# amazon-science/instruct-video-to-video

Hardware: AMD Instinct MI355X
Metric: denoised video-frames/sec (16f@256x384, 50 DDIM steps) (higher is better)
Workload: dtype fp16; 1 GPU; C2: 1 clip/step = VAE-encode + 50 DDIM steps (3-way CFG, text 7.5 / video 1.5) + VAE-decode, 16 frames @ 256x384, random-init full-width UNet+VAE; 5 independent clips in flight per GPU (stacked into every UNet launch, B = 3 x clips); frames=16, height=256, width=384, ddim_steps=50, clips_per_gpu=5, parallelism=clip-parallel x1, one all_gather, hip_graph=True, cfg_branch_streams=False, concurrent_clips=5, clip_mode=stacked, driver_mode=False, full=False

## Files before the change

### include/insv2v_hip.h

```cpp
#ifndef INSV2V_HIP_H
#define INSV2V_HIP_H

#include <stdint.h>

#ifdef __cplusplus
extern "C" {
#endif

typedef void* insv2v_stream_t;

#define INSV2V_OK 0
#define INSV2V_EINVAL (-1)
#define INSV2V_EUNSUPPORTED (-2)

#define INSV2V_ACT_NONE 0
#define INSV2V_ACT_SILU 1
#define INSV2V_ACT_GEGLU 2
#define INSV2V_ACT_QUICK_GELU 3

#define INSV2V_ACT_RELU 4
#define INSV2V_ACT_SIGMOID 5
#define INSV2V_ACT_TANH 6

#define INSV2V_MODE_LINEAR 0
// ... 26 lines not shown
    int32_t NB, IH, IW, OH, OW, Cin;
    int32_t stride, pad_t, pad_l, upsample;
    int32_t batch;
    int32_t tile;
    int32_t split_k;
    float alpha;
    const float* gn_ab;
    int32_t gn_images_per_sample;
    int32_t gn_silu;
    float* stats_out;
    float* stats_scratch;
    int32_t stats_parts;
    float ln_eps;
    int64_t w_group_stride;
    int32_t w_group_rows;
    int32_t reserved0;
} insv2v_gemm_desc;
int insv2v_gemm(const insv2v_gemm_desc* d, insv2v_stream_t stream);
int64_t insv2v_set_operand_window(int64_t bytes);
int insv2v_gemm_stats_parts(const insv2v_gemm_desc* d);
int insv2v_conv3x3_fuses_groupnorm(const insv2v_gemm_desc* d);
#define INSV2V_PLAN_NONE 0
#define INSV2V_PLAN_TILE 1
#define INSV2V_PLAN_HALO 2
#define INSV2V_PLAN_Q8 3
#define INSV2V_PLAN_R8 4
#define INSV2V_PLAN_W4 5
typedef struct insv2v_gemm_plan_t {
    int32_t rc;
    int32_t family;
    int32_t variant;
// ... 186 lines not shown
    int32_t grid;
    int32_t lds_bytes;
    int32_t rows_per_wg;
    int32_t ntiles;
    int32_t ragged;
} insv2v_attention_plan_t;
int insv2v_attention_plan(const insv2v_attention_desc* d, int32_t cus, insv2v_attention_plan_t* out);

int insv2v_embed_tokens(const int64_t* ids, const void* tok, const void* pos, void* out, int32_t rows, int32_t L,
                        int32_t C, int32_t vocab, insv2v_stream_t stream);

int insv2v_softmax_rows(const void* x, void* y, int64_t ldx, int64_t ldy, int32_t rows, int32_t cols,
                        float scale, insv2v_stream_t stream);
int insv2v_softmax_rows_padded(const void* x, void* y, int64_t ldx, int64_t ldy, int32_t rows, int32_t cols, int32_t valid,
                               float scale, insv2v_stream_t stream);

int insv2v_timestep_embedding(const float* t, void* out, int32_t batch, int32_t dim, float shift,
                              insv2v_stream_t stream);

int insv2v_tap_gather(const float* y9, int64_t ld9, const float* bias, float* out, int64_t ldo, int32_t NB, int32_t H, int32_t W,
                      int32_t cout, insv2v_stream_t stream);

int insv2v_build_unet_input(const float* latent, const float* img_cond, void* out, float* t_out,
                            float timestep, int32_t nbranch, int32_t F, int32_t h, int32_t w, int32_t ldo,
                            int64_t branch_rows, int32_t t_stride, insv2v_stream_t stream);

typedef struct insv2v_step_desc {
    const float* eps_in;
    const float* latent;
    const float* latent_ref;
// ... 251 lines not shown
```

### instruct-video-to-video_amd/csrc/gemm_plan.h

```cpp
#pragma once
#include <stdint.h>
#include <algorithm>
#include "../../include/insv2v_hip.h"

constexpr int GEMM_BK = 64;
constexpr int W4_BK = 32;

struct gemm_switches {
    int r8 = 1;
    int r8_stats = 1;
    int q8_min_n = 256;
    int persistent = 1;
    int r8_geglu = 1;
    int r8_cim = 1;
    int halo_legacy_map = 0;
    int r8_dephase = 0;
    int w4_wgs = 2, w4_delay = -1;
};
const gemm_switches& insv2v_gemm_switches();

static inline void gemm_defaults(insv2v_gemm_desc& d) { if (d.batch <= 0) d.batch = 1; if (d.alpha == 0.f) d.alpha = 1.f; }
static inline bool misaligned16(const void* p) { return ((uintptr_t)p & 15) != 0; }
static inline bool beyond_2g(int64_t bytes) { return bytes >= ((int64_t)1 << 31); }

// ... 146 lines not shown
    const int64_t nparts = (total + per - 1) / per;
    return ((total + nparts - 1) / nparts + unit - 1) / unit * unit;
}

static inline insv2v_gemm_desc window_part(const insv2v_gemm_desc& f, int64_t u0, int64_t nu) {
    const bool conv = f.mode == INSV2V_MODE_CONV3X3;
    const int64_t opix = conv ? (int64_t)f.OH * f.OW : 1, ipix = conv ? (int64_t)f.IH * f.IW : 1, esz = f.c_fp32 ? 4 : 2;
    const int64_t r_in = u0 * ipix, r_out = u0 * opix;
    insv2v_gemm_desc d = f;
    d.a = (const char*)f.a + r_in * f.lda * 2;
    if (f.k_split) d.a2 = (const char*)f.a2 + r_in * f.lda2 * 2;
    d.c = (char*)f.c + r_out * f.ldc * esz;
    if (f.residual) d.residual = (const char*)f.residual + r_out * f.ldr * 2;
    if (f.row_stats) d.row_stats = f.row_stats + r_out * 2;
    if (f.w_group_rows > 0) d.w = (const char*)f.w + (r_out / f.w_group_rows) * f.w_group_stride * 2;
    if (f.row_bias && f.rb_mod <= 0) d.row_bias = f.row_bias + (r_out / f.rows_per_group) * f.ld_rb;
    if (conv && f.gn_ab) d.gn_ab = f.gn_ab + (u0 / f.gn_images_per_sample) * (int64_t)f.Cin * 2;
    d.M = (int32_t)(nu * opix); if (conv) d.NB = (int32_t)nu;
    return d;
}
static inline void stats_finished(insv2v_gemm_desc& d) { d.row_stats = d.stats_scratch; d.stats_parts = 0; }

static inline int validate_gemm(const insv2v_gemm_desc& d, int stats_width) {
    if (!d.a || !d.w || !d.c || d.M <= 0 || d.N <= 0 || d.K <= 0) return INSV2V_EINVAL;
    if ((d.K & 7) || (d.lda & 7) || (d.ldw & 7)) return INSV2V_EINVAL;
    if (misaligned16(d.a) || misaligned16(d.w)) return INSV2V_EINVAL;
    if (d.k_split && (!d.a2 || (d.k_split % GEMM_BK) || (d.lda2 & 7) || misaligned16(d.a2))) return INSV2V_EINVAL;
    if (d.row_bias && d.rows_per_group <= 0) return INSV2V_EINVAL;
    if (d.row_stats && (!d.col_sum || d.batch > 1)) return INSV2V_EINVAL;
    if (d.stats_parts < 0 || (d.stats_parts > 0 && (!d.row_stats || !d.stats_scratch))) return INSV2V_EINVAL;
    if (d.stats_out && stats_width == 0) return INSV2V_EUNSUPPORTED;
    if (d.act == INSV2V_ACT_GEGLU && (d.N % 64)) return INSV2V_EINVAL;
    if (d.act < 0 || d.act > INSV2V_ACT_TANH) return INSV2V_EINVAL;
    if (d.w_group_rows < 0 || (d.w_group_rows > 0 && (d.w_group_rows % 256 || d.w_group_stride <= 0))) return INSV2V_EINVAL;
    if (d.w_group_rows > 0 && (d.mode != INSV2V_MODE_LINEAR || d.batch > 1 || d.c_fp32 || d.act != INSV2V_ACT_NONE || d.residual || d.row_bias || d.row_stats ||
                               d.stats_out || d.k_split || d.split_k > 1 || d.K < 256 || (d.N % 256 && d.N % 320)))
        return INSV2V_EUNSUPPORTED;
    if (d.gn_ab && (d.mode != INSV2V_MODE_CONV3X3 || d.gn_images_per_sample <= 0 || d.upsample)) return INSV2V_EINVAL;
    if (d.mode == INSV2V_MODE_CONV3X3) {
        if (d.Cin <= 0 || (d.Cin % GEMM_BK) || d.K != 9 * d.Cin) return INSV2V_EINVAL;
        if ((long)d.NB * d.OH * d.OW != d.M || d.stride < 1) return INSV2V_EINVAL;
        if (d.upsample && (d.stride != 1 || d.pad_t != 1 || d.pad_l != 1 || (d.OH != 2 * d.IH && d.OH != 2 * d.IH - 1) || (d.OW != 2 * d.IW && d.OW != 2 * d.IW - 1)))
            return INSV2V_EINVAL;
    } else if (d.mode != INSV2V_MODE_LINEAR) {
        return INSV2V_EUNSUPPORTED;
    }
    return beyond_2g((int64_t)d.N * d.ldw * 2) ? INSV2V_EUNSUPPORTED : 0;
}

static inline int engine_tile_code(int family) { return family == INSV2V_PLAN_R8 ? 240 : family == INSV2V_PLAN_Q8 ? 230 : 210; }
// ... 25 lines not shown
        const int64_t per = units_per_part(d, window), total = conv ? d.NB : d.M;
        if (per <= 0) return refuse(INSV2V_EUNSUPPORTED);
        const bool finalize = d.stats_parts > 0;
        if (finalize) stats_finished(d);
        const insv2v_gemm_plan_t first = plan_gemm(window_part(d, 0, per), cus, window, sw);
        if (first.rc) return refuse(first.rc);
        const int32_t stats_w_ = p.stats_width, fuse = p.gn_fuse;
        p = first;
        p.stats_width = stats_w_; p.gn_fuse = fuse; p.ln_finalize = finalize;
        p.parts = (int32_t)((total + per - 1) / per);
        p.units_per_part = (int32_t)per;
        return p;
    }
    if (d.w_group_rows > 0) {
        const int64_t groups = ((int64_t)d.M + d.w_group_rows - 1) / d.w_group_rows;
        if (beyond_2g(groups * d.w_group_stride * 2)) return refuse(INSV2V_EUNSUPPORTED);
        if (cus <= 0) return refuse(INSV2V_EINVAL);
        const bool r_ok = d.N % 320 == 0, q_ok = d.N % 256 == 0;
        const pingpong_cost c = pingpong_costs(d, cus);
        const bool use_r = d.tile / 10 == 24 ? true : d.tile / 10 == 23 ? false : (r_ok && (!q_ok || c.r8 <= c.q8));
        if (use_r ? !r_ok : !q_ok) return refuse(INSV2V_EUNSUPPORTED);
        if (const int rc = engine(use_r ? R8 : Q8)) return refuse(rc);
        return p;
    }
    if (d.tile >= 200 && d.tile <= 206) return refuse(INSV2V_EUNSUPPORTED);
    if ((d.tile >= 230 && d.tile <= 249) || (d.tile >= 210 && d.tile <= 221)) {
        const int family = d.tile >= 240 ? R8 : d.tile >= 230 ? Q8 : W4;
        if (d.split_k > 1 || (d.stats_out && family != R8)) return refuse(INSV2V_EUNSUPPORTED);
        d.split_k = 1;
        if (const int rc = engine(family, d.tile - engine_tile_code(family))) return refuse(rc);
        return p;
// ... 44 lines not shown
```

### instruct-video-to-video_amd/csrc/gemm_q8.hip

```cpp
#include "common.h"
#include "gemm_dma.h"
#include "gemm_plan.h"
#include <type_traits>

namespace {

constexpr int HALF_B = 128 * 128;
constexpr int RING_B = 8 * HALF_B;
constexpr int PARK_B = 5 * 1024;
constexpr int LDS_B = RING_B + 2 * PARK_B;
constexpr int STAMP_B = 8 * 512;

#ifndef Q8_MID_SPREAD
#define Q8_MID_SPREAD 1
#endif
#define SB() __builtin_amdgcn_sched_barrier(0)
#define BARRIER() do { SB(); __builtin_amdgcn_s_barrier(); SB(); } while (0)

typedef unsigned uint4v __attribute__((ext_vector_type(4)));
__device__ __forceinline__ unsigned pack_h2(float x, float y) {
    typedef float f2_t __attribute__((ext_vector_type(2)));
    const f2_t v = {x, y};
    return __builtin_bit_cast(unsigned, __builtin_convertvector(v, half2v));
}
// ... 102 lines not shown
    auto stage_piece = [&](auto part_c, auto buf_c, int i) {
        constexpr int PART = decltype(part_c)::value, BUF = decltype(buf_c)::value;
        char* dst = smem + (PART * 2 + BUF) * HALF_B + wid * 1024 + i * 8192;
        if (PART >= 2) dma16(rW, woff[(PART - 2) * 2 + i], cur.k0 * 2 + (int)cur.wbase, dst);
        else dma16(cur.second ? rA2 : rA, aoff[PART * 2 + i], cur.soffA, dst);
    };
    auto stage = [&](auto part_c, auto buf_c) { stage_piece(part_c, buf_c, 0); stage_piece(part_c, buf_c, 1); };
    auto row_group = [&](int m) { int g = m / p.rows_per_group; if (p.rb_mod > 0) g %= p.rb_mod; return g; };
    auto stage_park = [&](int pb, int bm0, int bn0) {
        char* dst = smem + RING_B + pb * PARK_B + wid * 1024;
        if (wid == 0) {
            const int n = bn0 + lane * 4;
            dma16(rBias, (p.bias && n < p.N) ? (unsigned)(n * 4) : OOB_OFFSET, 0, dst);
        } else if (wid == 1) {
            const int n = bn0 + lane * 4;
            dma16(rCs, (ln && n < p.N) ? (unsigned)(n * 4) : OOB_OFFSET, 0, dst);
        } else if (wid == 2 || wid == 3) {
            const int m = bm0 + (wid - 2) * 128 + lane * 2;
            dma16(rSt, (ln && m < p.M) ? (unsigned)(m * 8) : OOB_OFFSET, 0, dst);
        } else if (wid == 4) {
            const int n = bn0 + lane * 4;
            const int g = p.row_bias ? row_group(bm0) : 0;
            dma16(rRb, (p.row_bias && n < p.N) ? (unsigned)((g * (int)p.ld_rb + n) * 4) : OOB_OFFSET, 0, dst);
        }
    };

    const int l15 = lane & 15, lq = lane >> 4, fsw = l15 >> 1;
    const char* aRd[2];
    const char* wRd[2];
#pragma unroll
    for (int kb = 0; kb < 2; ++kb) {
// ... 292 lines not shown
```

### instruct-video-to-video_amd/csrc/gemm_r8.hip

```cpp
#include "common.h"
#include "gemm_dma.h"
#include "gemm_plan.h"
#include <type_traits>

namespace {

constexpr int BM = 256, BN = 320;
constexpr int AH_B = 128 * 128;
constexpr int WB_B = 64 * 128;
constexpr int W_BASE = 4 * AH_B;
constexpr int RING_B = 4 * AH_B + 10 * WB_B;
constexpr int PK_BIAS = 0, PK_CS = 2048, PK_ST = 4096, PK_RB = 6144, PARK_B = 8192;
constexpr int LDS_B = RING_B + 2 * PARK_B;

#ifndef R8_MID_SPREAD
#define R8_MID_SPREAD 1
#endif
#define SB() __builtin_amdgcn_sched_barrier(0)
#define BARRIER() do { SB(); __builtin_amdgcn_s_barrier(); SB(); } while (0)

typedef unsigned uint4v __attribute__((ext_vector_type(4)));
typedef unsigned uint2v __attribute__((ext_vector_type(2)));
__device__ __forceinline__ unsigned pack_h2(float x, float y) {
    typedef float f2_t __attribute__((ext_vector_type(2)));
// ... 155 lines not shown
        } else {
            dma16(rW, min(woff + (unsigned)(PB * 32 * (int)p.ldw * 2), wmax), cur.k0 * 2 + (int)cur.wbase, dst);
        }
    };
    auto row_group = [&](int m) { int g = m / p.rows_per_group; if (p.rb_mod > 0) g %= p.rb_mod; return g; };
    auto stage_park = [&](int pb, int bm0, int bn0) {
        char* park = smem + RING_B + pb * PARK_B;
        const srd_t rBias = make_srd(p.bias ? (const void*)p.bias : p.w), rCs = make_srd(ln ? (const void*)p.col_sum : p.w),
                    rSt = make_srd(ln ? (const void*)p.row_stats : p.w), rRb = make_srd(p.row_bias ? (const void*)p.row_bias : p.w);
        const int hi = wid & 1;
        const int n = bn0 + hi * 256 + lane * 4;
        const bool okn = n < p.N && (hi == 0 || lane < 16);
        if (wid < 2) {
            dma16(rBias, (p.bias && okn) ? (unsigned)(n * 4) : OOB_OFFSET, 0, park + PK_BIAS + hi * 1024);
        } else if (wid < 4) {
            dma16(rCs, (ln && okn) ? (unsigned)(n * 4) : OOB_OFFSET, 0, park + PK_CS + hi * 1024);
        } else if (wid < 6) {
            const int m = bm0 + hi * 128 + lane * 2;
            dma16(rSt, (ln && m < p.M) ? (unsigned)(m * 8) : OOB_OFFSET, 0, park + PK_ST + hi * 1024);
        } else {
            const int g = p.row_bias ? row_group(bm0) : 0;
            dma16(rRb, (p.row_bias && okn) ? (unsigned)((g * (int)p.ld_rb + n) * 4) : OOB_OFFSET, 0, park + PK_RB + hi * 1024);
        }
    };

    const int l15 = lane & 15, lq = lane >> 4, fsw = l15 >> 1;
    const char* aRd[2];
    const char* wRd[2];
#pragma unroll
    for (int kb = 0; kb < 2; ++kb) {
        const int co = ((kb * 4 + lq) ^ fsw) * 16;
// ... 356 lines not shown
```

### instruct-video-to-video_amd/csrc/norm.hip

```cpp
#include "common.h"
#include "norm_plan.h"
#include <cstdlib>

struct Moments {
    float n, mean, m2;
};
static_assert(sizeof(Moments) == GN_MOMENTS_BYTES, "norm_plan.h restates the size");
__device__ __forceinline__ Moments merge(Moments a, Moments b) {
    if (b.n == 0.f) return a;
    if (a.n == 0.f) return b;
    Moments r;
    r.n = a.n + b.n;
    float d = b.mean - a.mean;
    r.mean = a.mean + d * (b.n / r.n);
    r.m2 = a.m2 + b.m2 + d * d * (a.n * b.n / r.n);
    return r;
}

__device__ __forceinline__ half8 load8(const half_t* x, const half_t* x2, int64_t ldx, int64_t ldx2, int C1,
                                       int64_t row, int c0) {
    const half_t* p = (c0 < C1) ? x + row * ldx + c0 : x2 + row * ldx2 + (c0 - C1);
    return *(const half8*)p;
}

// ... 597 lines not shown
    if (!x || !y || rows <= 0 || cols <= 0 || (cols & 7) || (ldx & 7) || (ldy & 7)) return INSV2V_EINVAL;
    if (scale < 0.f) return INSV2V_EINVAL;
    hipLaunchKernelGGL(softmax_rows_kernel<false>, dim3(rows), dim3(256), 0, as_stream(stream), (const half_t*)x,
                       (half_t*)y, ldx, ldy, cols, cols, scale);
    return launch_status();
}

extern "C" int insv2v_softmax_rows_padded(const void* x, void* y, int64_t ldx, int64_t ldy, int32_t rows, int32_t cols, int32_t valid,
                                          float scale, insv2v_stream_t stream) {
    if (!x || !y || rows <= 0 || cols <= 0 || (cols & 7) || (ldx & 7) || (ldy & 7) || ldx < cols || ldy < cols) return INSV2V_EINVAL;
    if (valid <= 0 || valid > cols || scale < 0.f) return INSV2V_EINVAL;
    hipLaunchKernelGGL(softmax_rows_kernel<true>, dim3(rows), dim3(256), 0, as_stream(stream), (const half_t*)x,
                       (half_t*)y, ldx, ldy, cols, valid, scale);
    return launch_status();
}
```

### instruct-video-to-video_amd/insv2v/_lib.py

```python
import ctypes as C
import os

import torch

ABI_VERSION = 15
_HERE = os.path.dirname(os.path.abspath(__file__))
LIB_PATH = os.environ.get("INSV2V_LIB", os.path.join(_HERE, "libinsv2v_hip.so"))

c_i32, c_i64, c_f32, c_p = C.c_int32, C.c_int64, C.c_float, C.c_void_p


class GemmDesc(C.Structure):
    _fields_ = [("a", c_p), ("a2", c_p), ("w", c_p), ("c", c_p), ("bias", c_p), ("row_bias", c_p), ("residual", c_p),
                ("row_stats", c_p), ("col_sum", c_p),
                ("lda", c_i64), ("lda2", c_i64), ("ldw", c_i64), ("ldc", c_i64), ("ldr", c_i64), ("ld_rb", c_i64),
                ("a_bs", c_i64), ("w_bs", c_i64), ("c_bs", c_i64), ("r_bs", c_i64),
                ("workspace", c_p), ("workspace_bytes", c_i64),
                ("M", c_i32), ("N", c_i32), ("K", c_i32), ("k_split", c_i32), ("rows_per_group", c_i32),
                ("rb_mod", c_i32), ("act", c_i32), ("c_fp32", c_i32), ("mode", c_i32),
                ("NB", c_i32), ("IH", c_i32), ("IW", c_i32), ("OH", c_i32), ("OW", c_i32), ("Cin", c_i32),
                ("stride", c_i32), ("pad_t", c_i32), ("pad_l", c_i32), ("upsample", c_i32),
                ("batch", c_i32), ("tile", c_i32), ("split_k", c_i32), ("alpha", c_f32),
                ("gn_ab", c_p), ("gn_images_per_sample", c_i32), ("gn_silu", c_i32),
                ("stats_out", c_p), ("stats_scratch", c_p), ("stats_parts", c_i32), ("ln_eps", c_f32),
                ("w_group_stride", c_i64), ("w_group_rows", c_i32), ("reserved0", c_i32)]


class GemmPlan(C.Structure):
    _fields_ = [(n, c_i32) for n in ("rc", "family", "variant", "ring", "tw_shift", "cim", "split_k", "ln_finalize", "splitk_reduce", "stats_width",
                                     "gn_fuse", "parts", "units_per_part", "forced_tile")]


class WinogradInDesc(C.Structure):
    _fields_ = [("x", c_p), ("x2", c_p), ("gn_ab", c_p), ("v", c_p), ("ldx", c_i64), ("ldx2", c_i64), ("v_group_rows", c_i64),
                ("NB", c_i32), ("H", c_i32), ("W", c_i32), ("C", c_i32), ("C1", c_i32), ("gn_images_per_sample", c_i32), ("gn_silu", c_i32), ("upsample", c_i32)]


class WinogradOutDesc(C.Structure):
    _fields_ = [("m", c_p), ("bias", c_p), ("row_bias", c_p), ("residual", c_p), ("y", c_p), ("m_group_rows", c_i64),
                ("ldr", c_i64), ("ldy", c_i64), ("ld_rb", c_i64), ("NB", c_i32), ("H", c_i32), ("W", c_i32), ("Cout", c_i32), ("rows_per_group", c_i32), ("upsample", c_i32)]
# ... 151 lines not shown
    "insv2v_tattn_attn": (c_i32, [C.POINTER(TattnDesc), c_p]),
    "insv2v_tattn_attn_stream_elems": (c_i64, [c_i32, c_i32, c_i32]),
    "insv2v_xattn_fused": (c_i32, [C.POINTER(XattnDesc), c_p]),
    "insv2v_xattn_stream_elems": (c_i64, [c_i32, c_i32, c_i32]),
    "insv2v_xattn_attn": (c_i32, [C.POINTER(XattnDesc), c_p]),
    "insv2v_xattn_attn_stream_elems": (c_i64, [c_i32, c_i32, c_i32]),
    "insv2v_groupnorm": (c_i32, [C.POINTER(GroupNormDesc), c_p]),
    "insv2v_groupnorm_plan": (c_i32, [C.POINTER(GroupNormDesc), C.POINTER(GroupNormPlan)]),
    "insv2v_layernorm": (c_i32, [C.POINTER(LayerNormDesc), c_p]),
    "insv2v_layernorm_stats": (c_i32, [c_p, c_p, c_i64, c_i32, c_i32, c_f32, c_p]),
    "insv2v_attention": (c_i32, [C.POINTER(AttentionDesc), c_p]),
    "insv2v_attention_plan": (c_i32, [C.POINTER(AttentionDesc), c_i32, C.POINTER(AttentionPlan)]),
    "insv2v_embed_tokens": (c_i32, [c_p, c_p, c_p, c_p, c_i32, c_i32, c_i32, c_i32, c_p]),
    "insv2v_softmax_rows": (c_i32, [c_p, c_p, c_i64, c_i64, c_i32, c_i32, c_f32, c_p]),
    "insv2v_softmax_rows_padded": (c_i32, [c_p, c_p, c_i64, c_i64, c_i32, c_i32, c_i32, c_f32, c_p]),
    "insv2v_timestep_embedding": (c_i32, [c_p, c_p, c_i32, c_i32, c_f32, c_p]),
    "insv2v_build_unet_input": (c_i32, [c_p, c_p, c_p, c_p, c_f32, c_i32, c_i32, c_i32, c_i32, c_i32, c_i64, c_i32, c_p]),
    "insv2v_cfg_step": (c_i32, [C.POINTER(StepDesc), c_p]),
    "insv2v_cfg_step_ms": (c_i32, [C.POINTER(MStepDesc), c_p]),
    "insv2v_cfg_step_mask": (c_i32, [C.POINTER(MaskStepDesc), c_p]),
    "insv2v_mask_to_latent": (c_i32, [c_p, c_p, c_i32, c_i32, c_i32, c_i32, c_p]),
    "insv2v_composite": (c_i32, [c_p, c_p, c_p, c_p, c_i32, c_i32, c_i32, c_p]),
    "insv2v_add_noise": (c_i32, [c_p, c_p, c_p, c_i64, c_f32, c_f32, c_p]),
    "insv2v_cfg_stats": (c_i32, [c_p, c_p, c_i32, c_i32, c_i32, c_f32, c_f32, c_i64, c_p]),
    "insv2v_warp_image": (c_i32, [c_p, c_p, c_p, c_i32, c_i32, c_i32, c_i32, c_p]),
    "insv2v_tap_gather": (c_i32, [c_p, c_i64, c_p, c_p, c_i64, c_i32, c_i32, c_i32, c_i32, c_p]),
    "insv2v_resize_flow": (c_i32, [c_p, c_p, c_i32, c_i32, c_i32, c_i32, c_i32, c_p]),
    "insv2v_flow_correction": (c_i32, [c_p, c_p, c_p, c_p, c_p, c_i32, c_i32, c_i32, c_i32, c_f32, c_f32, c_p]),
    "insv2v_nchw_to_nhwc_f16": (c_i32, [c_p, c_p, c_i32, c_i32, c_i32, c_i32, c_i32, c_f32, c_p]),
    "insv2v_nhwc_to_nchw_f32": (c_i32, [c_p, c_i32, c_p, c_i32, c_i32, c_i32, c_i32, c_i32, c_f32, c_p]),
# ... 60 lines not shown
```

### instruct-video-to-video_amd/insv2v/inference.py

```python
import os
import weakref

import torch

from . import ops
from .fused import check_operand_windows
from .rng import stream_id, STEP, MASK, WINDOW_BITS, STEP_BITS
from .schedulers import DDIMScheduler, DDPMScheduler, DPMSolverMultistepScheduler, strength_to_start
from .flow_utils import resize_flow


class GraphedUNet:

    def __init__(self, unet, B, F, H, W, ctx_len, use_graph=True, branch_streams=False, cfg_clips=0):
        dev = unet.device
        self.branch_streams = branch_streams and B > 1
        self.cfg_clips = cfg_clips if (cfg_clips > 0 and B == 3 * cfg_clips and not self.branch_streams) else 0
        self._streams = None
        try:
            self._unet = weakref.ref(unet)
        except TypeError:
            self._unet = lambda u=unet: u
        self.key = (B, F, H, W, ctx_len)
        self.x_in = torch.zeros((B * F * H * W, unet.in_pad), device=dev, dtype=torch.float16)
# ... 4 lines not shown
        self.eps = None
        self.start = 0
        self._ws = [ops.new_workspace(dev) for _ in range(B if self.branch_streams else 1)]

    @property
    def unet(self):
        u = self._unet()
        if u is None:
            raise RuntimeError("GraphedUNet: its UNet has been garbage collected")
        return u

    def set_context(self, ctx):
        kvs, L = self.unet.project_context(ctx)
        assert L == self.key[4] and ctx.shape[0] == self.key[0]
        if self.kvs is None:
            self.kvs = [tuple(torch.zeros_like(t) for t in kv) if isinstance(kv, tuple) else torch.zeros_like(kv) for kv in kvs]
        for dst, src in zip(self.kvs, kvs):
            for d, s_ in zip(dst, src) if isinstance(dst, tuple) else ((dst, src),):
                d.copy_(s_)

    def _forward(self):
        B, F, H, W, L = self.key
        if not self.branch_streams:
            with ops.workspace(self._ws[0]):
                return self.unet.forward_cl(self.x_in, self.t, self.kvs, L, B, F, H, W, start=self.start, cfg_clips=self.cfg_clips)
        if self._streams is None:
            self._streams = [torch.cuda.Stream() for _ in range(B)]
        main = torch.cuda.current_stream()
        rows = F * H * W
        outs = [None] * B
        for b, st in enumerate(self._streams):
            st.wait_stream(main)
            with torch.cuda.stream(st), ops.workspace(self._ws[b]):
                kvs = [(kv[0][b * L:(b + 1) * L], kv[1][b:b + 1]) if isinstance(kv, tuple) else kv[b * L:(b + 1) * L] for kv in self.kvs]
                outs[b] = self.unet.forward_cl(self.x_in[b * rows:(b + 1) * rows], self.t[b:b + 1], kvs, L, 1, F, H, W,
                                               start=self.start)
        for st in self._streams:
            main.wait_stream(st)
        return torch.cat(outs, 0)

    def run(self):
        if not self.use_graph:
            return self._forward()
        if self.graph is None:
            s = torch.cuda.Stream()
            s.wait_stream(torch.cuda.current_stream())
            with torch.cuda.stream(s):
                self._forward()
            torch.cuda.current_stream().wait_stream(s)
# ... 567 lines not shown
```

### instruct-video-to-video_amd/insv2v/ops.py

```python
import ctypes as C

import math
import os
import torch

from . import _lib
from .rng import as_int64
from ._lib import GemmDesc, GroupNormDesc, LayerNormDesc, AttentionDesc, StepDesc, MStepDesc, MaskStepDesc, MaskTrackDesc, FfnDesc, RowLinDesc, TattnDesc, XattnDesc, WinogradInDesc, WinogradOutDesc, check

ACT_NONE, ACT_SILU, ACT_GEGLU, ACT_QUICK_GELU = 0, 1, 2, 3
ACT_RELU, ACT_SIGMOID, ACT_TANH = 4, 5, 6
EW_RELU, EW_ADD_RELU, EW_TANH, EW_GRU_RH, EW_GRU_OUT = 1, 2, 3, 4, 5
_byref = C.byref


def _stream():
    return torch.cuda.current_stream().cuda_stream


_REC = None


def set_launch_recorder(rec):
    global _REC
# ... 66 lines not shown


class RowStats:
    __slots__ = ("parts", "nparts", "eps")

    def __init__(self, parts, nparts, eps):
        self.parts, self.nparts, self.eps = parts, nparts, eps


_STATS_PARTS_CACHE = {}


def gemm(a, w, bias=None, *, a2=None, act=ACT_NONE, residual=None, row_bias=None, rows_per_group=0, rb_mod=0,
         row_stats=None, col_sum=None, emit_stats=False, ln_eps=1e-5,
         out=None, out_fp32=False, alpha=1.0, tile=0, split_k=0, batch=1, a_bs=0, w_bs=0, c_bs=0, r_bs=0,
         M=None, N=None, K=None, lda=None, ldw=None, ldc=None):
    lib = _lib.load()
    _req(a, torch.float16, "gemm.a"), _req(w, torch.float16, "gemm.w")
    M = a.shape[0] if M is None else M
    N = w.shape[0] if N is None else N
    k1 = a.shape[1]
    K = (k1 + (a2.shape[1] if a2 is not None else 0)) if K is None else K
    n_out = N // 2 if act == ACT_GEGLU else N
    if out is None:
        shape = (M, n_out) if batch == 1 else (batch, M, n_out)
        out = torch.empty(shape, device=a.device, dtype=torch.float32 if out_fp32 else torch.float16)
    d = GemmDesc()
    d.a, d.w, d.c = a.data_ptr(), w.data_ptr(), out.data_ptr()
    d.lda = a.stride(0) if lda is None else lda
    d.ldw = w.stride(0) if ldw is None else ldw
    d.ldc = (out.stride(-2) if ldc is None else ldc)
# ... 7 lines not shown
    if residual is not None:
        d.residual, d.ldr = _req(residual, torch.float16, "gemm.residual").data_ptr(), residual.stride(-2)
    scratch = None
    if isinstance(row_stats, RowStats):
        d.row_stats = row_stats.parts.data_ptr()
        d.stats_parts, d.ln_eps = row_stats.nparts, row_stats.eps
        scratch = torch.empty((M, 2), device=a.device, dtype=torch.float32)
        d.stats_scratch = scratch.data_ptr()
        d.col_sum = _req(col_sum, torch.float32, "gemm.col_sum").data_ptr()
    elif row_stats is not None:
        d.row_stats = _req(row_stats, torch.float32, "gemm.row_stats").data_ptr()
        d.col_sum = _req(col_sum, torch.float32, "gemm.col_sum").data_ptr()
    d.rb_mod = rb_mod
    d.M, d.N, d.K, d.act, d.c_fp32, d.alpha, d.tile = M, N, K, act, int(out.dtype == torch.float32), alpha, tile
    d.batch, d.a_bs, d.w_bs, d.c_bs, d.r_bs = batch, a_bs, w_bs, c_bs, r_bs
    if batch == 1:
        ws = _workspace(a.device)
        d.workspace, d.workspace_bytes, d.split_k = ws.data_ptr(), ws.numel() * 4, split_k
    stats = None
    if emit_stats:
        key = (M, N, K, d.lda, d.ldc, d.ldr, residual is not None, act, tile, out.dtype, a.data_ptr() % 16, out.data_ptr() % 16, batch, split_k,
               residual.data_ptr() % 16 if residual is not None else 0,
               row_bias is not None, rows_per_group, d.ld_rb, rb_mod, a2 is not None, row_stats is not None)
        nparts = _STATS_PARTS_CACHE.get(key)
        if nparts is None:
            nparts = _STATS_PARTS_CACHE[key] = int(lib.insv2v_gemm_stats_parts(_byref(d)))
        if nparts > 0:
            stats = RowStats(torch.empty((nparts, M, 2), device=a.device, dtype=torch.float32), nparts, ln_eps)
            d.stats_out = stats.parts.data_ptr()
    with _timed("gemm_kernel", 2.0 * M * N * K * batch, ("lin", M, N, K, batch, act, residual is not None)):
        rc = lib.insv2v_gemm(_byref(d), _stream())
        if rc == -2 and stats is not None:
            stats, d.stats_out = None, None
            rc = lib.insv2v_gemm(_byref(d), _stream())
        check(rc, "insv2v_gemm")
    del scratch
    if emit_stats:
        return out, (stats if stats is not None else layernorm_stats(out, ln_eps))
# ... 436 lines not shown


def softmax_rows(x, scale=1.0, valid=None):
    lib = _lib.load()
    _req(x, torch.float16, "softmax.x")
    x2 = x.reshape(-1, x.shape[-1])
    if valid is not None and valid != x2.shape[1]:
        check(lib.insv2v_softmax_rows_padded(x2.data_ptr(), x2.data_ptr(), x2.stride(0), x2.stride(0), x2.shape[0], x2.shape[1], valid,
                                             scale, _stream()), "insv2v_softmax_rows_padded")
        return x
    check(lib.insv2v_softmax_rows(x2.data_ptr(), x2.data_ptr(), x2.stride(0), x2.stride(0), x2.shape[0], x2.shape[1],
                                  scale, _stream()), "insv2v_softmax_rows")
    return x


def timestep_embedding(t_dev, dim, shift=0.0):
    lib = _lib.load()
    _req(t_dev, torch.float32, "timestep")
    out = torch.empty((t_dev.shape[0], dim), device=t_dev.device, dtype=torch.float16)
    check(lib.insv2v_timestep_embedding(t_dev.data_ptr(), out.data_ptr(), t_dev.shape[0], dim, shift, _stream()),
          "insv2v_timestep_embedding")
    return out


def build_unet_input(latent, img_cond, out, t_out, timestep, nbranch, branch_rows=0, t_stride=0):
    lib = _lib.load()
    F, _, h, w = latent.shape[-4:]
    check(lib.insv2v_build_unet_input(_req(latent, torch.float32, "latent").data_ptr(),
                                      _req(img_cond, torch.float32, "img_cond").data_ptr(), out.data_ptr(),
                                      _ptr(t_out), float(timestep), nbranch, F, h, w, out.shape[-1], branch_rows, t_stride, _stream()),
# ... 587 lines not shown
```

### instruct-video-to-video_amd/insv2v/unet.py

```python
import math
import os

import torch

from . import ops
from . import fused
from .fused import check_operand_windows, pack_ffn_stream, pack_linear_stream, pack_tattn_stream, pack_tattn_qkv_stream

CPAD = 64
FUSE_GN = os.environ.get("INSV2V_FUSE_GN", "0") != "0"
FUSE_FFN = os.environ.get("INSV2V_FUSE_FFN", "1") != "0"
FUSE_FFN_POST = os.environ.get("INSV2V_FUSE_FFN_POST", "1") != "0"
DEDUP_CFG = os.environ.get("INSV2V_DEDUP_CFG", "1") != "0"
WINOGRAD = os.environ.get("INSV2V_WINOGRAD", "1") != "0"
WINOGRAD_MIN_CIN = int(os.environ.get("INSV2V_WINOGRAD_MIN_CIN", "1280"))
WINOGRAD_MIN_ROWS = int(os.environ.get("INSV2V_WINOGRAD_MIN_ROWS", "4608"))
WINOGRAD_UP_MIN_CIN = int(os.environ.get("INSV2V_WINOGRAD_UP_MIN_CIN", "640"))
MERGE_FF2_POST = os.environ.get("INSV2V_MERGE_FF2_POST", "1") != "0"
NARROW_CONV_OUT = os.environ.get("INSV2V_NARROW_CONV_OUT", "1") != "0"
NARROW_CONV_MIN_ROWS = int(os.environ.get("INSV2V_NARROW_CONV_MIN_ROWS", "16384"))
ROWLIN = os.environ.get("INSV2V_ROWLIN", "1") != "0"
ROWLIN_640 = os.environ.get("INSV2V_ROWLIN_640", "1") != "0"
ROWLIN_640_MIN_ROWS = int(os.environ.get("INSV2V_ROWLIN_640_MIN_ROWS", "55296"))

# ... 176 lines not shown
        self.ff = FeedForwardW(sd, b + ".ff", device, b + ".norm3", post_key=key + ".proj_out")
        self.rl = None
        if ROWLIN and ops.rowlin_supported(ch, ch) and (ch != 640 or ROWLIN_640):
            lin = lambda k: (sd[k + ".weight"], sd[k + ".bias"])
            self.rl = dict(proj_in=rowlin_stream(*lin(key + ".proj_in"), device), proj_out=rowlin_stream(*lin(key + ".proj_out"), device),
                           qkv=rowlin_stream(self.wqkv.float(), self.qkv_b, device), wo1=rowlin_stream(*lin(f"{b}.attn1.to_out.0"), device),
                           q2=rowlin_stream(self.wq2.float(), self.q2_b, device), wo2=rowlin_stream(*lin(f"{b}.attn2.to_out.0"), device))
        self.xa_stream, self.xa640_stream, self.xa_pre_stream = None, None, None
        if self.rl is not None and FUSE_XATTN and ops.xattn_fused_supported(ch, heads, 77, 128):
            self.xa_stream = fused.pack_xattn_stream(self.wq2.float(), self.q2_b, *lin(f"{b}.attn2.to_out.0")).to(device)
            if FUSE_XATTN_PRE:
                self.xa_pre_stream = fused.pack_xattn_stream(self.wq2.float(), self.q2_b, *lin(f"{b}.attn2.to_out.0"),
                                                             pre=lin(f"{b}.attn1.to_out.0")).to(device)
        elif self.rl is not None and FUSE_XATTN_640 and ops.xattn_attn_supported(ch, heads, 77, 128):
            self.xa640_stream = fused.pack_xattn_q_stream(self.wq2.float(), self.q2_b).to(device)

    def project_context(self, ctx2d, ctx_len=0):
        kv = ops.gemm(ctx2d, self.wkv2)
        if self.xa_stream is not None and ctx_len and 64 < ctx_len <= 96:
            return kv, fused.pack_xattn_kv(kv, kv.shape[0] // ctx_len, ctx_len, self.ch, self.heads)
        if self.xa640_stream is not None and ctx_len and 64 < ctx_len <= 96:
            return kv, fused.pack_xattn640_kv(kv, kv.shape[0] // ctx_len, ctx_len, self.ch, self.heads)
        return kv

    def __call__(self, x, kv, ctx_len, shared=0):
        C, hd, BF, HW = self.ch, self.ch // self.heads, x.B * x.F, x.hw
        scale = hd ** -0.5
        rl = self.rl if (C != 640 or _rowlin_640_pays(x.t.shape[0])) else None
        a = None
        if rl is not None and ROWLIN_GN and shared > 0 and x.B == 3 * shared:
            r1, r2 = shared * x.F * HW, 2 * shared * x.F * HW
            ab = ops.groupnorm_stats(x.t[:r2], 2 * shared * x.F, HW, *self.norm, self.groups, 1e-6)
            h, st = torch.empty((x.t.shape[0], C), device=x.t.device, dtype=torch.float16), None
# ... 12 lines not shown
            qkv = ops.rowlin(h, rl["qkv"], 3 * C, layernorm=True)
        elif rl is not None:
            n = ops.groupnorm(x.t, BF, HW, *self.norm, self.groups, 1e-6)
            h, st = ops.rowlin(n, rl["proj_in"], C), None
            qkv = ops.rowlin(h, rl["qkv"], 3 * C, layernorm=True)
        else:
            n = ops.groupnorm(x.t, BF, HW, *self.norm, self.groups, 1e-6)
            h, st = ops.gemm(n, *self.proj_in, emit_stats=True)
            qkv = ops.gemm(h, self.wqkv, self.qkv_b, row_stats=st, col_sum=self.qkv_cs)
        if a is None:
            a = torch.empty((x.t.shape[0], C), device=h.device, dtype=torch.float16)
            p = qkv.data_ptr()
            ops.attention(p, p + 2 * C, p + 4 * C, a, batch=BF, heads=self.heads, head_dim=hd, seq_q=HW, seq_k=HW,
                          scale=scale, q_rs=3 * C, k_rs=3 * C, v_rs=3 * C, o_rs=C,
                          q_addr=(1, HW * 3 * C, 0), kv_addr=(1, HW * 3 * C, 0), o_addr=(1, HW * C, 0))
        kv, kv_frag = kv if isinstance(kv, tuple) else (kv, None)
        if rl is None:
            kv_frag = None
        xa = kv_frag is not None and ops.xattn_fused_supported(C, self.heads, ctx_len, x.F * HW)
        if xa:
            if self.xa_pre_stream is not None and h.is_contiguous():
                h2 = ops.xattn_fused(a, self.xa_pre_stream, kv_frag, x.F * HW, self.heads, ctx_len, pre_residual=h)
            else:
                h = ops.rowlin(a, rl["wo1"], C, residual=h)
                h2 = ops.xattn_fused(h, self.xa_stream, kv_frag, x.F * HW, self.heads, ctx_len)
            if self.ff.stream_post is not None:
                return x.like(self.ff.with_proj_out(h2, x.t))
            h = self.ff(h2, None) if self.ff.stream is not None else self.ff(h2, h2, ops.layernorm_stats(h2))
            return x.like(ops.rowlin(h, rl["proj_out"], C, residual=x.t))
        if kv_frag is not None and self.xa640_stream is not None and ops.xattn_attn_supported(C, self.heads, ctx_len, x.F * HW):
# ... 384 lines not shown
```

Measured before the change: 16.50 frames/s.

## Fold prompt K/V into Q and out projections for cross-attention

Adds a per-prompt algebraic fold of cross-attention. K·Wq and V·Wo are precomputed once per context, so each block's Q projection, attention and out projection become two grouped GEMMs around a new segmented softmax kernel. The grouped-weight GEMM path gains per-group col_sum offsets, so the LayerNorm stats trick keeps working across clips. It applies only to non-rowlin blocks where heads×80 fits within half the channels (the 1280-channel blocks). It adds per-prompt precompute cost and fp16 rounding of the folded weights.

```diff
diff --git a/include/insv2v_hip.h b/include/insv2v_hip.h
--- a/include/insv2v_hip.h
+++ b/include/insv2v_hip.h
@@ -64,7 +64,7 @@
     float ln_eps;
     int64_t w_group_stride;
     int32_t w_group_rows;
-    int32_t reserved0;
+    int32_t cs_group_stride;
 } insv2v_gemm_desc;
 int insv2v_gemm(const insv2v_gemm_desc* d, insv2v_stream_t stream);
 int64_t insv2v_set_operand_window(int64_t bytes);
@@ -281,6 +281,7 @@
                         float scale, insv2v_stream_t stream);
 int insv2v_softmax_rows_padded(const void* x, void* y, int64_t ldx, int64_t ldy, int32_t rows, int32_t cols, int32_t valid,
                                float scale, insv2v_stream_t stream);
+int insv2v_softmax_segments(void* x, int64_t ld, int32_t rows, int32_t nseg, int32_t seg, int32_t valid, insv2v_stream_t stream);
 
 int insv2v_timestep_embedding(const float* t, void* out, int32_t batch, int32_t dim, float shift,
                               insv2v_stream_t stream);
diff --git a/instruct-video-to-video_amd/csrc/gemm_plan.h b/instruct-video-to-video_amd/csrc/gemm_plan.h
--- a/instruct-video-to-video_amd/csrc/gemm_plan.h
+++ b/instruct-video-to-video_amd/csrc/gemm_plan.h
@@ -184,6 +184,7 @@
     if (f.residual) d.residual = (const char*)f.residual + r_out * f.ldr * 2;
     if (f.row_stats) d.row_stats = f.row_stats + r_out * 2;
     if (f.w_group_rows > 0) d.w = (const char*)f.w + (r_out / f.w_group_rows) * f.w_group_stride * 2;
+    if (f.w_group_rows > 0 && f.cs_group_stride > 0 && f.col_sum) d.col_sum = f.col_sum + (r_out / f.w_group_rows) * f.cs_group_stride;
     if (f.row_bias && f.rb_mod <= 0) d.row_bias = f.row_bias + (r_out / f.rows_per_group) * f.ld_rb;
     if (conv && f.gn_ab) d.gn_ab = f.gn_ab + (u0 / f.gn_images_per_sample) * (int64_t)f.Cin * 2;
     d.M = (int32_t)(nu * opix); if (conv) d.NB = (int32_t)nu;
@@ -203,7 +204,9 @@
     if (d.act == INSV2V_ACT_GEGLU && (d.N % 64)) return INSV2V_EINVAL;
     if (d.act < 0 || d.act > INSV2V_ACT_TANH) return INSV2V_EINVAL;
     if (d.w_group_rows < 0 || (d.w_group_rows > 0 && (d.w_group_rows % 256 || d.w_group_stride <= 0))) return INSV2V_EINVAL;
-    if (d.w_group_rows > 0 && (d.mode != INSV2V_MODE_LINEAR || d.batch > 1 || d.c_fp32 || d.act != INSV2V_ACT_NONE || d.residual || d.row_bias || d.row_stats ||
+    if (d.cs_group_stride < 0 || (d.cs_group_stride > 0 && (d.w_group_rows <= 0 || (d.cs_group_stride & 3)))) return INSV2V_EINVAL;
+    if (d.w_group_rows > 0 && (d.mode != INSV2V_MODE_LINEAR || d.batch > 1 || d.c_fp32 || d.act != INSV2V_ACT_NONE ||
+                               (d.cs_group_stride == 0 && (d.residual || d.row_bias || d.row_stats)) ||
                                d.stats_out || d.k_split || d.split_k > 1 || d.K < 256 || (d.N % 256 && d.N % 320)))
         return INSV2V_EUNSUPPORTED;
     if (d.gn_ab && (d.mode != INSV2V_MODE_CONV3X3 || d.gn_images_per_sample <= 0 || d.upsample)) return INSV2V_EINVAL;
@@ -259,7 +262,7 @@
     }
     if (d.w_group_rows > 0) {
         const int64_t groups = ((int64_t)d.M + d.w_group_rows - 1) / d.w_group_rows;
-        if (beyond_2g(groups * d.w_group_stride * 2)) return refuse(INSV2V_EUNSUPPORTED);
+        if (beyond_2g(groups * d.w_group_stride * 2) || beyond_2g(groups * d.cs_group_stride * 4)) return refuse(INSV2V_EUNSUPPORTED);
         if (cus <= 0) return refuse(INSV2V_EINVAL);
         const bool r_ok = d.N % 320 == 0, q_ok = d.N % 256 == 0;
         const pingpong_cost c = pingpong_costs(d, cus);
diff --git a/instruct-video-to-video_amd/csrc/gemm_q8.hip b/instruct-video-to-video_amd/csrc/gemm_q8.hip
--- a/instruct-video-to-video_amd/csrc/gemm_q8.hip
+++ b/instruct-video-to-video_amd/csrc/gemm_q8.hip
@@ -140,7 +140,8 @@
             dma16(rBias, (p.bias && n < p.N) ? (unsigned)(n * 4) : OOB_OFFSET, 0, dst);
         } else if (wid == 1) {
             const int n = bn0 + lane * 4;
-            dma16(rCs, (ln && n < p.N) ? (unsigned)(n * 4) : OOB_OFFSET, 0, dst);
+            const int cso = (MODE == INSV2V_MODE_LINEAR && p.w_group_rows > 0) ? (bm0 / p.w_group_rows) * p.cs_group_stride * 4 : 0;
+            dma16(rCs, (ln && n < p.N) ? (unsigned)(n * 4) : OOB_OFFSET, cso, dst);
         } else if (wid == 2 || wid == 3) {
             const int m = bm0 + (wid - 2) * 128 + lane * 2;
             dma16(rSt, (ln && m < p.M) ? (unsigned)(m * 8) : OOB_OFFSET, 0, dst);
diff --git a/instruct-video-to-video_amd/csrc/gemm_r8.hip b/instruct-video-to-video_amd/csrc/gemm_r8.hip
--- a/instruct-video-to-video_amd/csrc/gemm_r8.hip
+++ b/instruct-video-to-video_amd/csrc/gemm_r8.hip
@@ -193,7 +193,8 @@
         if (wid < 2) {
             dma16(rBias, (p.bias && okn) ? (unsigned)(n * 4) : OOB_OFFSET, 0, park + PK_BIAS + hi * 1024);
         } else if (wid < 4) {
-            dma16(rCs, (ln && okn) ? (unsigned)(n * 4) : OOB_OFFSET, 0, park + PK_CS + hi * 1024);
+            const int cso = (LIN && p.w_group_rows > 0) ? (bm0 / p.w_group_rows) * p.cs_group_stride * 4 : 0;
+            dma16(rCs, (ln && okn) ? (unsigned)(n * 4) : OOB_OFFSET, cso, park + PK_CS + hi * 1024);
         } else if (wid < 6) {
             const int m = bm0 + hi * 128 + lane * 2;
             dma16(rSt, (ln && m < p.M) ? (unsigned)(m * 8) : OOB_OFFSET, 0, park + PK_ST + hi * 1024);
diff --git a/instruct-video-to-video_amd/csrc/norm.hip b/instruct-video-to-video_amd/csrc/norm.hip
--- a/instruct-video-to-video_amd/csrc/norm.hip
+++ b/instruct-video-to-video_amd/csrc/norm.hip
@@ -635,3 +635,56 @@
                        (half_t*)y, ldx, ldy, cols, valid, scale);
     return launch_status();
 }
+
+constexpr int SEG_U = 4;
+__global__ __launch_bounds__(256) void softmax_segments_kernel(half_t* x, int64_t ld, int64_t items, int nseg, int seg8, int valid) {
+    const int sub = threadIdx.x & 15;
+    const int64_t g0 = ((int64_t)blockIdx.x * 16 + (threadIdx.x >> 4)) * SEG_U;
+    half_t* ptr[SEG_U];
+    bool live[SEG_U];
+    half8 v[SEG_U];
+#pragma unroll
+    for (int u = 0; u < SEG_U; ++u) {
+        const int64_t item = g0 + u, row = item / nseg;
+        const int s = (int)(item - row * nseg);
+        live[u] = item < items && sub < seg8;
+        ptr[u] = x + row * ld + (s * seg8 + sub) * 8;
+        if (live[u]) v[u] = *(const half8*)ptr[u];
+    }
+#pragma unroll
+    for (int u = 0; u < SEG_U; ++u) {
+        float f[8], mx = -3.0e38f;
+#pragma unroll
+        for (int e = 0; e < 8; ++e) {
+            const bool ok = live[u] && sub * 8 + e < valid;
+            f[e] = ok ? (float)v[u][e] : -3.0e38f;
+            mx = fmaxf(mx, f[e]);
+        }
+#pragma unroll
+        for (int o = 8; o > 0; o >>= 1) mx = fmaxf(mx, __shfl_xor(mx, o, 64));
+        float sum = 0.f;
+#pragma unroll
+        for (int e = 0; e < 8; ++e) {
+            f[e] = (live[u] && sub * 8 + e < valid) ? exp2f((f[e] - mx) * 1.4426950408889634f) : 0.f;
+            sum += f[e];
+        }
+#pragma unroll
+        for (int o = 8; o > 0; o >>= 1) sum += __shfl_xor(sum, o, 64);
+        if (live[u]) {
+            const float inv = 1.f / sum;
+            half8 o8;
+#pragma unroll
+            for (int e = 0; e < 8; ++e) o8[e] = (half_t)(f[e] * inv);
+            *(half8*)ptr[u] = o8;
+        }
+    }
+}
+
+extern "C" int insv2v_softmax_segments(void* x, int64_t ld, int32_t rows, int32_t nseg, int32_t seg, int32_t valid, insv2v_stream_t stream) {
+    if (!x || rows <= 0 || nseg <= 0 || seg <= 0 || (seg & 7) || seg > 128 || valid <= 0 || valid > seg) return INSV2V_EINVAL;
+    if ((ld & 7) || ld < (int64_t)nseg * seg || ((uintptr_t)x & 15)) return INSV2V_EINVAL;
+    const int64_t items = (int64_t)rows * nseg, per_wg = 16 * SEG_U, wgs = (items + per_wg - 1) / per_wg;
+    if (wgs > 0x7fffffff) return INSV2V_EUNSUPPORTED;
+    hipLaunchKernelGGL(softmax_segments_kernel, dim3((unsigned)wgs), dim3(256), 0, as_stream(stream), (half_t*)x, ld, items, nseg, seg / 8, valid);
+    return launch_status();
+}
diff --git a/instruct-video-to-video_amd/insv2v/_lib.py b/instruct-video-to-video_amd/insv2v/_lib.py
--- a/instruct-video-to-video_amd/insv2v/_lib.py
+++ b/instruct-video-to-video_amd/insv2v/_lib.py
@@ -23,7 +23,7 @@
                 ("batch", c_i32), ("tile", c_i32), ("split_k", c_i32), ("alpha", c_f32),
                 ("gn_ab", c_p), ("gn_images_per_sample", c_i32), ("gn_silu", c_i32),
                 ("stats_out", c_p), ("stats_scratch", c_p), ("stats_parts", c_i32), ("ln_eps", c_f32),
-                ("w_group_stride", c_i64), ("w_group_rows", c_i32), ("reserved0", c_i32)]
+                ("w_group_stride", c_i64), ("w_group_rows", c_i32), ("cs_group_stride", c_i32)]
 
 
 class GemmPlan(C.Structure):
@@ -205,6 +205,7 @@
     "insv2v_embed_tokens": (c_i32, [c_p, c_p, c_p, c_p, c_i32, c_i32, c_i32, c_i32, c_p]),
     "insv2v_softmax_rows": (c_i32, [c_p, c_p, c_i64, c_i64, c_i32, c_i32, c_f32, c_p]),
     "insv2v_softmax_rows_padded": (c_i32, [c_p, c_p, c_i64, c_i64, c_i32, c_i32, c_i32, c_f32, c_p]),
+    "insv2v_softmax_segments": (c_i32, [c_p, c_i64, c_i32, c_i32, c_i32, c_i32, c_p]),
     "insv2v_timestep_embedding": (c_i32, [c_p, c_p, c_i32, c_i32, c_f32, c_p]),
     "insv2v_build_unet_input": (c_i32, [c_p, c_p, c_p, c_p, c_f32, c_i32, c_i32, c_i32, c_i32, c_i32, c_i64, c_i32, c_p]),
     "insv2v_cfg_step": (c_i32, [C.POINTER(StepDesc), c_p]),
diff --git a/instruct-video-to-video_amd/insv2v/inference.py b/instruct-video-to-video_amd/insv2v/inference.py
--- a/instruct-video-to-video_amd/insv2v/inference.py
+++ b/instruct-video-to-video_amd/insv2v/inference.py
@@ -5,6 +5,7 @@
 
 from . import ops
 from .fused import check_operand_windows
+from .xattn_fold import FoldedContext
 from .rng import stream_id, STEP, MASK, WINDOW_BITS, STEP_BITS
 from .schedulers import DDIMScheduler, DDPMScheduler, DPMSolverMultistepScheduler, strength_to_start
 from .flow_utils import resize_flow
@@ -42,7 +43,7 @@
         kvs, L = self.unet.project_context(ctx)
         assert L == self.key[4] and ctx.shape[0] == self.key[0]
         if self.kvs is None:
-            self.kvs = [tuple(torch.zeros_like(t) for t in kv) if isinstance(kv, tuple) else torch.zeros_like(kv) for kv in kvs]
+            self.kvs = [type(kv)(torch.zeros_like(t) for t in kv) if isinstance(kv, tuple) else torch.zeros_like(kv) for kv in kvs]
         for dst, src in zip(self.kvs, kvs):
             for d, s_ in zip(dst, src) if isinstance(dst, tuple) else ((dst, src),):
                 d.copy_(s_)
@@ -60,7 +61,8 @@
         for b, st in enumerate(self._streams):
             st.wait_stream(main)
             with torch.cuda.stream(st), ops.workspace(self._ws[b]):
-                kvs = [(kv[0][b * L:(b + 1) * L], kv[1][b:b + 1]) if isinstance(kv, tuple) else kv[b * L:(b + 1) * L] for kv in self.kvs]
+                kvs = [kv.sample(b, L) if isinstance(kv, FoldedContext) else (kv[0][b * L:(b + 1) * L], kv[1][b:b + 1]) if isinstance(kv, tuple)
+                       else kv[b * L:(b + 1) * L] for kv in self.kvs]
                 outs[b] = self.unet.forward_cl(self.x_in[b * rows:(b + 1) * rows], self.t[b:b + 1], kvs, L, 1, F, H, W,
                                                start=self.start)
         for st in self._streams:
diff --git a/instruct-video-to-video_amd/insv2v/ops.py b/instruct-video-to-video_amd/insv2v/ops.py
--- a/instruct-video-to-video_amd/insv2v/ops.py
+++ b/instruct-video-to-video_amd/insv2v/ops.py
@@ -104,7 +104,7 @@
 def gemm(a, w, bias=None, *, a2=None, act=ACT_NONE, residual=None, row_bias=None, rows_per_group=0, rb_mod=0,
          row_stats=None, col_sum=None, emit_stats=False, ln_eps=1e-5,
          out=None, out_fp32=False, alpha=1.0, tile=0, split_k=0, batch=1, a_bs=0, w_bs=0, c_bs=0, r_bs=0,
-         M=None, N=None, K=None, lda=None, ldw=None, ldc=None):
+         M=None, N=None, K=None, lda=None, ldw=None, ldc=None, w_group_rows=0, w_group_stride=0, cs_group_stride=0):
     lib = _lib.load()
     _req(a, torch.float16, "gemm.a"), _req(w, torch.float16, "gemm.w")
     M = a.shape[0] if M is None else M
@@ -142,6 +142,7 @@
     d.rb_mod = rb_mod
     d.M, d.N, d.K, d.act, d.c_fp32, d.alpha, d.tile = M, N, K, act, int(out.dtype == torch.float32), alpha, tile
     d.batch, d.a_bs, d.w_bs, d.c_bs, d.r_bs = batch, a_bs, w_bs, c_bs, r_bs
+    d.w_group_rows, d.w_group_stride, d.cs_group_stride = w_group_rows, w_group_stride, cs_group_stride
     if batch == 1:
         ws = _workspace(a.device)
         d.workspace, d.workspace_bytes, d.split_k = ws.data_ptr(), ws.numel() * 4, split_k
@@ -149,7 +150,7 @@
     if emit_stats:
         key = (M, N, K, d.lda, d.ldc, d.ldr, residual is not None, act, tile, out.dtype, a.data_ptr() % 16, out.data_ptr() % 16, batch, split_k,
                residual.data_ptr() % 16 if residual is not None else 0,
-               row_bias is not None, rows_per_group, d.ld_rb, rb_mod, a2 is not None, row_stats is not None)
+               row_bias is not None, rows_per_group, d.ld_rb, rb_mod, a2 is not None, row_stats is not None, w_group_rows)
         nparts = _STATS_PARTS_CACHE.get(key)
         if nparts is None:
             nparts = _STATS_PARTS_CACHE[key] = int(lib.insv2v_gemm_stats_parts(_byref(d)))
@@ -616,6 +617,16 @@
     return x
 
 
+def softmax_segments(x, nseg, seg, valid):
+    lib = _lib.load()
+    _req(x, torch.float16, "softmax_segments.x")
+    if x.dim() != 2 or x.stride(1) != 1:
+        raise _lib.HipKernelError("softmax_segments: expected a row-major matrix")
+    with _timed("layernorm", 0.0, ("ln", x.shape[0], nseg * seg)):
+        check(lib.insv2v_softmax_segments(x.data_ptr(), x.stride(0), x.shape[0], nseg, seg, valid, _stream()), "insv2v_softmax_segments")
+    return x
+
+
 def timestep_embedding(t_dev, dim, shift=0.0):
     lib = _lib.load()
     _req(t_dev, torch.float32, "timestep")
diff --git a/instruct-video-to-video_amd/insv2v/unet.py b/instruct-video-to-video_amd/insv2v/unet.py
--- a/instruct-video-to-video_amd/insv2v/unet.py
+++ b/instruct-video-to-video_amd/insv2v/unet.py
@@ -5,6 +5,7 @@
 
 from . import ops
 from . import fused
+from . import xattn_fold
 from .fused import check_operand_windows, pack_ffn_stream, pack_linear_stream, pack_tattn_stream, pack_tattn_qkv_stream
 
 CPAD = 64
@@ -214,9 +215,12 @@
                                                              pre=lin(f"{b}.attn1.to_out.0")).to(device)
         elif self.rl is not None and FUSE_XATTN_640 and ops.xattn_attn_supported(ch, heads, 77, 128):
             self.xa640_stream = fused.pack_xattn_q_stream(self.wq2.float(), self.q2_b).to(device)
+        self.fold = xattn_fold.PromptFold(self.wq2, self.q2_b, self.wo2[0], heads) if (self.rl is None and xattn_fold.fold_supported(ch, heads, 77, True)) else None
 
     def project_context(self, ctx2d, ctx_len=0):
         kv = ops.gemm(ctx2d, self.wkv2)
+        if self.fold is not None and xattn_fold.fold_supported(self.ch, self.heads, ctx_len):
+            return self.fold(kv, ctx_len)
         if self.xa_stream is not None and ctx_len and 64 < ctx_len <= 96:
             return kv, fused.pack_xattn_kv(kv, kv.shape[0] // ctx_len, ctx_len, self.ch, self.heads)
         if self.xa640_stream is not None and ctx_len and 64 < ctx_len <= 96:
@@ -259,6 +263,17 @@
             ops.attention(p, p + 2 * C, p + 4 * C, a, batch=BF, heads=self.heads, head_dim=hd, seq_q=HW, seq_k=HW,
                           scale=scale, q_rs=3 * C, k_rs=3 * C, v_rs=3 * C, o_rs=C,
                           q_addr=(1, HW * 3 * C, 0), kv_addr=(1, HW * 3 * C, 0), o_addr=(1, HW * C, 0))
+        folded = None
+        if isinstance(kv, xattn_fold.FoldedContext):
+            folded, kv = (kv if xattn_fold.fold_applies(C, self.heads, ctx_len, x.F * HW) else None), kv[0]
+        if folded is not None and rl is None:
+            h, st = ops.gemm(a, *self.wo1, residual=h, emit_stats=True)
+            h = xattn_fold.forward(h, st, folded, self.heads, ctx_len, x.F * HW, self.wo2[1])
+            st = ops.layernorm_stats(h)
+            if self.ff.w2p is not None:
+                return x.like(self.ff.with_proj_out_gemm(h, st, x.t))
+            h = self.ff(h, h, st)
+            return x.like(ops.gemm(h, *self.proj_out, residual=x.t))
         kv, kv_frag = kv if isinstance(kv, tuple) else (kv, None)
         if rl is None:
             kv_frag = None
diff --git a/instruct-video-to-video_amd/insv2v/xattn_fold.py b/instruct-video-to-video_amd/insv2v/xattn_fold.py
--- /dev/null
+++ b/instruct-video-to-video_amd/insv2v/xattn_fold.py
@@ -0,0 +1,77 @@
+import os
+
+import torch
+
+from . import ops
+
+XATTN_FOLD = os.environ.get("INSV2V_XATTN_FOLD", "1") != "0"
+CTX_PAD = 80
+
+
+def fold_supported(C, heads, ctx_len, enabled=None):
+    if not (XATTN_FOLD if enabled is None else enabled):
+        return False
+    if heads <= 0 or C % heads or (C // heads) % 8 or not 0 < ctx_len <= CTX_PAD:
+        return False
+    n1 = heads * CTX_PAD
+    return n1 <= C // 2 and n1 % 64 == 0 and C % 64 == 0 and (n1 % 320 == 0 or n1 % 256 == 0) and (C % 320 == 0 or C % 256 == 0)
+
+
+def fold_applies(C, heads, ctx_len, rows_per_sample, enabled=None):
+    return fold_supported(C, heads, ctx_len, enabled) and rows_per_sample > 0 and rows_per_sample % 256 == 0
+
+
+def fold_math(k, v, wq, q_bias, wo, heads, scale, pad=CTX_PAD):
+    S, L, C = k.shape
+    d = C // heads
+    kh, vh = k.reshape(S, L, heads, d), v.reshape(S, L, heads, d)
+    A = k.new_zeros(S, heads, pad, C)
+    b1 = k.new_zeros(S, heads, pad)
+    B = k.new_zeros(S, heads, pad, C)
+    A[:, :, :L] = scale * torch.einsum("slhc,hck->shlk", kh, wq.reshape(heads, d, C))
+    b1[:, :, :L] = scale * torch.einsum("slhc,hc->shl", kh, q_bias.reshape(heads, d))
+    B[:, :, :L] = torch.einsum("slhc,nhc->shln", vh, wo.reshape(C, heads, d))
+    return A.reshape(S, heads * pad, C), b1.reshape(S, heads * pad), B.reshape(S, heads * pad, C)
+
+
+class FoldedContext(tuple):
+
+    def sample(self, b, L):
+        kv, A, cs, b1, W2 = self
+        n1, C = cs.shape[1], A.shape[1]
+        return FoldedContext((kv[b * L:(b + 1) * L], A[b * n1:(b + 1) * n1], cs[b:b + 1], b1[b:b + 1], W2[b * C:(b + 1) * C]))
+
+
+class PromptFold:
+
+    def __init__(self, wq, q_bias, wo, heads):
+        self.C, self.heads = wq.shape[0], heads
+        self.wq_t = wq.t().contiguous()
+        self.q_bias, self.wo = q_bias, wo
+
+    def __call__(self, kv, L):
+        C, H, P = self.C, self.heads, CTX_PAD
+        d, S, n1 = C // H, kv.shape[0] // L, H * CTX_PAD
+        scale = d ** -0.5
+        A32 = torch.zeros((S, n1, C), device=kv.device, dtype=torch.float32)
+        B32 = torch.zeros((S, n1, C), device=kv.device, dtype=torch.float32)
+        for h in range(H):
+            cols = slice(h * d, (h + 1) * d)
+            kw = dict(batch=S, a_bs=L * 2 * C, c_bs=n1 * C, M=L, N=C, K=d)
+            ops.gemm(kv[:, cols], self.wq_t[:, cols], out=A32[:, h * P:h * P + L], alpha=scale, **kw)
+            ops.gemm(kv[:, C + h * d:C + (h + 1) * d], self.wo[:, cols], out=B32[:, h * P:h * P + L], **kw)
+        A = A32.half()
+        cs = A.float().sum(-1)
+        b1 = torch.zeros((S, H, P), device=kv.device, dtype=torch.float32)
+        b1[:, :, :L] = scale * torch.einsum("slhc,hc->shl", kv[:, :C].float().reshape(S, L, H, d), self.q_bias.reshape(H, d))
+        W2 = B32.transpose(1, 2).half().contiguous()
+        return FoldedContext((kv, A.reshape(S * n1, C), cs, b1.reshape(S, n1), W2.reshape(S * C, n1)))
+
+
+def forward(h, st, fc, heads, ctx_len, rows_per_sample, out_bias):
+    _, A, cs, b1, W2 = fc
+    C, n1 = A.shape[1], cs.shape[1]
+    s = ops.gemm(h, A, None, row_bias=b1, rows_per_group=rows_per_sample, row_stats=st, col_sum=cs, N=n1, K=C,
+                 w_group_rows=rows_per_sample, w_group_stride=n1 * C, cs_group_stride=n1)
+    ops.softmax_segments(s, heads, CTX_PAD, ctx_len)
+    return ops.gemm(s, W2, out_bias, residual=h, N=C, K=n1, w_group_rows=rows_per_sample, w_group_stride=C * n1, cs_group_stride=C)
```

Result: no change. 16.60 frames/s, median of 6 (+0.6%).
